# arcosoph/nanowakeword

Hardware: AMD Instinct MI355X
Metric: clips/sec (1 s @16 kHz PCM->logits) (higher is better)
Workload: dtype f32; 1 GPU; cnn head on (101,64) log-mel, batch=4096/GPU, 1 s 16 kHz mono int16 clips, 64-mel 25 ms/10 ms center frontend, fused STFT+mel HIP kernel, fp32; clips_per_gpu=4096, n_samples=16000, parallelism=batch-split x1

## Files before the change

### nanowakeword_amd/csrc/gemm_x3.hip

```cpp
#include <hip/hip_runtime.h>
#include <stdint.h>
#include <stdlib.h>
#include "layers.h"
#include "split_h2.h"

typedef float f32x16 __attribute__((ext_vector_type(16)));
typedef __bf16 bf16x8 __attribute__((ext_vector_type(8)));
typedef _Float16 f16x8 __attribute__((ext_vector_type(8)));
typedef _Float16 f16x2 __attribute__((ext_vector_type(2)));
typedef float f32x2 __attribute__((ext_vector_type(2)));
typedef float f32x4v __attribute__((ext_vector_type(4)));
typedef uint32_t u32x4v __attribute__((ext_vector_type(4)));

#ifdef X3_TRACE
__device__ unsigned long long x3_trace_buf[4 * 16 * 4];
#define X3_STAMP(kt_rel, ph)                                                                                        \
    if (blockIdx.x == 0 && blockIdx.y == 0 && blockIdx.z == 0 && (kt_rel) < 16 && (threadIdx.x & 63) == 0)        \
        x3_trace_buf[((threadIdx.x >> 6) * 16 + (kt_rel)) * 4 + (ph)] = __builtin_readcyclecounter();
#else
#define X3_STAMP(kt_rel, ph)
#endif
namespace {
constexpr int X3_BM = 128;
template <bool H2> struct X3A { static constexpr int NT = H2 ? 2 : 3, ROW = 64 * NT + 16; };

__device__ __forceinline__ float x3_sigmoid(float v) {
    return __builtin_amdgcn_rcpf(1.0f + __builtin_amdgcn_exp2f(-1.4426950408889634f * v));
}
template <int ACT>
__device__ __forceinline__ float x3_act(float v) {
    if (ACT == ACT_RELU) return fmaxf(v, 0.0f);
    if (ACT == ACT_GELU) return nww_gelu(v);
    if (ACT == ACT_SILU) return v * x3_sigmoid(v);
    if (ACT == ACT_SIGMOID) return x3_sigmoid(v);
    return v;
}

__device__ __forceinline__ void split3(float x, uint32_t& hi, uint32_t& mid, uint32_t& lo) {
    hi = __float_as_uint(x) & 0xffff0000u;
    const float r = x - __uint_as_float(hi);
    mid = __float_as_uint(r) & 0xffff0000u;
    lo = __float_as_uint(r - __uint_as_float(mid));
}
__device__ __forceinline__ uint32_t pack_hi16(uint32_t a, uint32_t b) { return __builtin_amdgcn_perm(b, a, 0x07060302u); }
template <bool H2>
__device__ __forceinline__ void x3_products(const uint4* a, const uint4* w, f32x16& acc) {
    if (H2) {
        const f16x8 ah = __builtin_bit_cast(f16x8, a[0]), al = __builtin_bit_cast(f16x8, a[1]);
        const f16x8 wh = __builtin_bit_cast(f16x8, w[0]), wl = __builtin_bit_cast(f16x8, w[1]);
        acc = __builtin_amdgcn_mfma_f32_32x32x16_f16(al, wh, acc, 0, 0, 0);
        acc = __builtin_amdgcn_mfma_f32_32x32x16_f16(ah, wl, acc, 0, 0, 0);
        acc = __builtin_amdgcn_mfma_f32_32x32x16_f16(ah, wh, acc, 0, 0, 0);
    } else {
        const bf16x8 ah = __builtin_bit_cast(bf16x8, a[0]), am = __builtin_bit_cast(bf16x8, a[1]), al = __builtin_bit_cast(bf16x8, a[H2 ? 1 : 2]);
        const bf16x8 wh = __builtin_bit_cast(bf16x8, w[0]), wm = __builtin_bit_cast(bf16x8, w[1]), wl = __builtin_bit_cast(bf16x8, w[H2 ? 1 : 2]);
        acc = __builtin_amdgcn_mfma_f32_32x32x16_bf16(am, wm, acc, 0, 0, 0);
        acc = __builtin_amdgcn_mfma_f32_32x32x16_bf16(ah, wl, acc, 0, 0, 0);
        acc = __builtin_amdgcn_mfma_f32_32x32x16_bf16(al, wh, acc, 0, 0, 0);
        acc = __builtin_amdgcn_mfma_f32_32x32x16_bf16(ah, wm, acc, 0, 0, 0);
        acc = __builtin_amdgcn_mfma_f32_32x32x16_bf16(am, wh, acc, 0, 0, 0);
        acc = __builtin_amdgcn_mfma_f32_32x32x16_bf16(ah, wh, acc, 0, 0, 0);
    }
}
}

__global__ void __launch_bounds__(256) split_weights_x3_kernel(const float* __restrict__ W, uint16_t* __restrict__ out,
                                                               int N, int K, int KB) {
    const size_t idx = (size_t)blockIdx.x * 256 + threadIdx.x;
    const size_t total = (size_t)N * KB * 16;
    if (idx >= total) return;
    const int kk = (int)(idx & 15);
    const size_t nb = idx >> 4;
    const int kb = (int)(nb % KB), n = (int)(nb / KB);
    const int k = kb * 16 + kk;
    const float x = k < K ? W[(size_t)n * K + k] : 0.0f;
    uint32_t hi, mid, lo;
    split3(x, hi, mid, lo);
    uint16_t* o = out + nb * 48 + kk;
    o[0] = (uint16_t)(hi >> 16); o[16] = (uint16_t)(mid >> 16); o[32] = (uint16_t)(lo >> 16);
}

__global__ void __launch_bounds__(256) split_weights_h2_kernel(const float* __restrict__ W, uint16_t* __restrict__ out,
                                                               int N, int K, int KB, float scale) {
    const size_t idx = (size_t)blockIdx.x * 256 + threadIdx.x;
    const size_t total = (size_t)N * KB * 16;
    if (idx >= total) return;
    const int kk = (int)(idx & 15);
    const size_t nb = idx >> 4;
    const int kb = (int)(nb % KB), n = (int)(nb / KB);
    const int k = kb * 16 + kk;
    const float x = k < K ? W[(size_t)n * K + k] * scale : 0.0f;
    uint32_t hi, lo;
    nww_split2h(x, 0.0f, hi, lo);
    uint16_t* o = out + nb * 32 + kk;
    o[0] = (uint16_t)hi; o[16] = (uint16_t)lo;
}

template <int CB, int NST, int ACT, bool H2>
__global__ void __launch_bounds__(256) __attribute__((amdgpu_num_vgpr(184))) gemm_x3_kernel(GemmArgs g) {
    constexpr int NT = X3A<H2>::NT, X3_ROW = X3A<H2>::ROW, PB = 2 * NT;
    { float agpr_hint = 0.0f; asm volatile("; mfma accumulators in AGPRs" : "+a"(agpr_hint)); }
    constexpr int BN = 32 * CB;
    constexpr int WPIECES = BN * 2 * PB;
    constexpr int WLD = (WPIECES + 255) / 256;
    extern __shared__ __attribute__((aligned(16))) unsigned char smem[];
    auto As = [&](int) { return smem; };
    auto Ws = [&](int) { return smem + X3_BM * X3_ROW; };
    const int tid = threadIdx.x, lane = tid & 63, wave = tid >> 6;
    const int i = lane & 31, h = lane >> 5;
    const int bxi = blockIdx.x, byi = blockIdx.y, bzi = blockIdx.z;
    const int bm = bxi * X3_BM, bn = byi * BN;
    const int KT = (g.K + 31) >> 5, KB = 2 * KT;
    int kt_begin = 0, kt_end = KT;
    if (g.splitk > 1) {
        const int kc = (KT + g.splitk - 1) / g.splitk;
        kt_begin = bzi * kc;
        kt_end = min(KT, kt_begin + kc);
    }
    const uint4* Wx = reinterpret_cast<const uint4*>(g.Wx3);

    const int lr = tid >> 3, lq = tid & 7;
    const float* arow[4];
#pragma unroll
    for (int q = 0; q < 4; ++q)
        arow[q] = g.a_blocked ? g.A + ((size_t)(bm >> 7) * g.a_blocked * 128 + lr + 32 * q) * 32 + 4 * lq
                              : g.A + (size_t)min(bm + lr + 32 * q, g.M - 1) * g.lda + 4 * lq;
    const int a_kstep = g.a_blocked ? 128 * 32 : 32;
    constexpr int AQ = (NST > 1 && CB == 1) ? 2 : 4;
    struct Stage { f32x4v a[AQ]; u32x4v w[WLD]; };
    auto gload = [&](int kt, Stage& st) {
        const int k = kt * 32 + 4 * lq;
        const size_t a_off = k + 4 <= g.K ? (size_t)kt * a_kstep : 0;
#pragma unroll
        for (int q = 0; q < AQ; ++q) {
            st.a[q] = *reinterpret_cast<const f32x4v*>(arow[q] + a_off);
        }
#pragma unroll
        for (int j = 0; j < WLD; ++j) {
            const int p = tid + 256 * j;
            if (WPIECES % 256 == 0 || p < WPIECES) {
                const int row = p / (2 * PB), c = p - row * (2 * PB);
                const int n = min(bn + row, g.N - 1);
                const int kb = 2 * kt + c / PB;
                st.w[j] = *reinterpret_cast<const u32x4v*>(Wx + ((size_t)n * KB + kb) * PB + (c % PB));
            }
        }
    };
    const float a_scale = H2 ? g.a_scale : 1.0f;
    const float a_lim = H2 ? (g.a_clamp > 0.0f ? g.a_clamp * a_scale : 65504.0f) : 0.0f;
    auto lstore = [&](int buf, const Stage& st) {
#pragma unroll
        for (int q = 0; q < AQ; ++q) {
            unsigned char* d = As(buf) + (lr + 32 * q) * X3_ROW + 8 * lq;
            if (H2) {
                uint32_t h0, l0, h1, l1;
                nww_split2h(__builtin_amdgcn_fmed3f(st.a[q][0] * a_scale, -a_lim, a_lim), __builtin_amdgcn_fmed3f(st.a[q][1] * a_scale, -a_lim, a_lim), h0, l0);
                nww_split2h(__builtin_amdgcn_fmed3f(st.a[q][2] * a_scale, -a_lim, a_lim), __builtin_amdgcn_fmed3f(st.a[q][3] * a_scale, -a_lim, a_lim), h1, l1);
                *reinterpret_cast<uint2*>(d) = make_uint2(h0, h1);
                *reinterpret_cast<uint2*>(d + 64) = make_uint2(l0, l1);
            } else {
                uint32_t hi[4], mid[4], lo[4];
                split3(st.a[q][0], hi[0], mid[0], lo[0]); split3(st.a[q][1], hi[1], mid[1], lo[1]);
                split3(st.a[q][2], hi[2], mid[2], lo[2]); split3(st.a[q][3], hi[3], mid[3], lo[3]);
                *reinterpret_cast<uint2*>(d) = make_uint2(pack_hi16(hi[0], hi[1]), pack_hi16(hi[2], hi[3]));
                *reinterpret_cast<uint2*>(d + 64) = make_uint2(pack_hi16(mid[0], mid[1]), pack_hi16(mid[2], mid[3]));
                *reinterpret_cast<uint2*>(d + 128) = make_uint2(pack_hi16(lo[0], lo[1]), pack_hi16(lo[2], lo[3]));
            }
        }
#pragma unroll
        for (int j = 0; j < WLD; ++j) {
            const int p = tid + 256 * j;
            if (WPIECES % 256 == 0 || p < WPIECES) {
                const int row = p / (2 * PB), c = p - row * (2 * PB);
                const int cp = c % PB;
                *reinterpret_cast<u32x4v*>(Ws(buf) + row * X3_ROW + (cp >> 1) * 64 + (c / PB) * 32 + (cp & 1) * 16) = st.w[j];
            }
        }
    };

    f32x16 acc[CB];
#pragma unroll
    for (int c = 0; c < CB; ++c)
#pragma unroll
        for (int r = 0; r < 16; ++r) acc[c][r] = 0.0f;

    Stage st[NST];
#pragma unroll
    for (int q = 0; q < NST; ++q) gload(min(kt_begin + q, kt_end - 1), st[q]);
    const bool has_rows = bm + wave * 32 < g.M;
    const int a_off = (wave * 32 + i) * X3_ROW + 16 * h, w_off = i * X3_ROW + 16 * h;
    auto multiply = [&]() {
#pragma unroll
        for (int kk = 0; kk < 2; ++kk) {
            const unsigned char* ap = As(0) + a_off + 32 * kk;
            uint4 af[NT];
#pragma unroll
            for (int t = 0; t < NT; ++t) af[t] = *reinterpret_cast<const uint4*>(ap + 64 * t);
#pragma unroll
            for (int c = 0; c < CB; ++c) {
                const unsigned char* wp = Ws(0) + w_off + c * 32 * X3_ROW + 32 * kk;
                uint4 wf[NT];
#pragma unroll
                for (int t = 0; t < NT; ++t) wf[t] = *reinterpret_cast<const uint4*>(wp + 64 * t);
                x3_products<H2>(af, wf, acc[c]);
            }
        }
    };
    for (int kt = kt_begin; kt < kt_end; kt += NST) {
#pragma unroll
        for (int q = 0; q < NST; ++q) {
            if (kt + q < kt_end) {
                X3_STAMP(kt + q - kt_begin, 0)
                __syncthreads();
                X3_STAMP(kt + q - kt_begin, 1)
                lstore(0, st[q]);
                __syncthreads();
                X3_STAMP(kt + q - kt_begin, 2)
            }
            gload(min(kt + q + NST, kt_end - 1), st[q]);
            if (kt + q < kt_end && (NST == 1 || has_rows)) multiply();
            X3_STAMP(kt + q - kt_begin, 3)
        }
    }

    const int m0 = bm + wave * 32;
    if (m0 >= g.M) return;
    if (H2) {
        const float c_scale = g.c_scale;
#pragma unroll
        for (int c = 0; c < CB; ++c)
#pragma unroll
            for (int r = 0; r < 16; ++r) acc[c][r] *= c_scale;
    }
#pragma unroll
    for (int c = 0; c < CB; ++c) {
        const int n = bn + c * 32 + i;
        if (n >= g.N) continue;
        if (g.splitk > 1) {
            float* part = g.splitk_ws + (size_t)bzi * g.M * g.N;
#pragma unroll
            for (int r = 0; r < 16; ++r) {
                const int m = m0 + (r & 3) + 8 * (r >> 2) + 4 * h;
                if (m < g.M) part[(size_t)m * g.N + n] = acc[c][r];
            }
            continue;
        }
        const float bias = g.bias ? g.bias[n] : 0.0f;
        const float al2 = g.alpha ? g.alpha[n] : 1.0f, be2 = g.alpha ? g.beta[n] : 0.0f;
        float* cp = g.C + (size_t)(m0 + 4 * h) * g.ldc + n;
        const float* rp = g.res ? g.res + (size_t)(m0 + 4 * h) * g.ldres + n : nullptr;
        const bool full = m0 + 32 <= g.M;
        auto finish = [&](float a) {
            float v = a + bias;
            v = v * al2 + be2;
            return x3_act<ACT>(v);
        };
        if (full && !rp) {
#pragma unroll
            for (int r = 0; r < 16; ++r) cp[(size_t)((r & 3) + 8 * (r >> 2)) * g.ldc] = finish(acc[c][r]);
        } else if (full) {
#pragma unroll
            for (int r = 0; r < 16; ++r) {
                const size_t ro = (size_t)((r & 3) + 8 * (r >> 2));
                cp[ro * g.ldc] = rp[ro * g.ldres] + g.rscale * finish(acc[c][r]);
            }
        } else {
#pragma unroll
            for (int r = 0; r < 16; ++r) {
                const int mo = (r & 3) + 8 * (r >> 2);
                if (m0 + 4 * h + mo < g.M) {
                    float v = finish(acc[c][r]);
                    if (rp) v = rp[(size_t)mo * g.ldres] + g.rscale * v;
                    cp[(size_t)mo * g.ldc] = v;
                }
            }
        }
    }
}

constexpr int CH_NW = 8, CH_TPW = 4;
template <bool H2>
__global__ void __launch_bounds__(64 * CH_NW) gemm_x3_chain_kernel(GemmArgs g) {
    constexpr int NT = X3A<H2>::NT, PB = 2 * NT;
    const float a_scale = H2 ? g.a_scale : 1.0f, c_scale = H2 ? g.c_scale : 1.0f;
    const float a_lim = H2 ? (g.a_clamp > 0.0f ? g.a_clamp * a_scale : 65504.0f) : 0.0f;
    __shared__ __attribute__((aligned(16))) float4 hand[4 * 64];
    const int lane = threadIdx.x & 63, wave = __builtin_amdgcn_readfirstlane((int)(threadIdx.x >> 6));
    const int i = lane & 31, h = lane >> 5;
    const int bm = blockIdx.x * 32, bn = blockIdx.y * 32;
    const int KT = (g.K + 31) >> 5, KB = 2 * KT;
    const int kc = (KT + g.splitk - 1) / g.splitk;
    const int kt_begin = blockIdx.z * kc, kt_end = min(KT, kt_begin + kc);
    const int mrow = min(bm + i, g.M - 1);
    const uint4* wrow = reinterpret_cast<const uint4*>(g.Wx3) + (size_t)min(bn + i, g.N - 1) * KB * PB + h;
    const float* abase = g.a_blocked ? g.A + ((size_t)(mrow >> 7) * g.a_blocked * 128 + (mrow & 127)) * 32 + 8 * h
                                     : g.A + (size_t)mrow * g.lda + 8 * h;
    const size_t a_kstep = g.a_blocked ? 128 * 32 : 32;

    f32x16 acc;
#pragma unroll
    for (int r = 0; r < 16; ++r) acc[r] = 0.0f;
    if (kt_begin >= kt_end) {
        if (wave == 0 && bn + i < g.N) {
            float* part = g.splitk_ws + (size_t)blockIdx.z * g.M * g.N;
#pragma unroll
            for (int r = 0; r < 16; ++r) {
// ... 84 lines not shown

hipError_t launch_split_weights_h2(const float* W, void* out, int N, int K, float scale, hipStream_t s) {
    const int KB = 2 * ((K + 31) / 32);
    const size_t total = (size_t)N * KB * 16;
    hipLaunchKernelGGL(split_weights_h2_kernel, dim3((unsigned)((total + 255) / 256)), dim3(256), 0, s, W,
                       reinterpret_cast<uint16_t*>(out), N, K, KB, scale);
    return hipGetLastError();
}

hipError_t launch_split_weights_x3(const float* W, void* out, int N, int K, hipStream_t s) {
    const int KB = 2 * ((K + 31) / 32);
    const size_t total = (size_t)N * KB * 16;
    hipLaunchKernelGGL(split_weights_x3_kernel, dim3((unsigned)((total + 255) / 256)), dim3(256), 0, s, W,
                       reinterpret_cast<uint16_t*>(out), N, K, KB);
    return hipGetLastError();
}

static int x3_pick_cb(int N) {
    int best = 2;
    long best_cost = -1;
    for (int cb = 2; cb <= 6; ++cb) {
        const long tiles = (N + 32 * cb - 1) / (32 * cb);
        const long cost = tiles * 32 * cb * 8 - cb;
        if (best_cost < 0 || cost < best_cost) { best_cost = cost; best = cb; }
    }
    return best;
}

bool gemm_x3_usable(const GemmArgs& g) {
    return g.Wx3 != nullptr && g.N >= 32 && g.K >= 32 && (g.K % 4 == 0) && (g.lda % 4 == 0) && (!g.a_blocked || g.K % 32 == 0) &&
           ((reinterpret_cast<uintptr_t>(g.A) & 15) == 0);
}

hipError_t launch_gemm_x3(const GemmArgs& g, hipStream_t s) {
    const int sk = (g.splitk > 1 && g.splitk_ws) ? g.splitk : 1;
    GemmArgs a = g;
    a.splitk = sk;
    const bool h2 = a.h2 != 0;
    const size_t row_b = h2 ? X3A<true>::ROW : X3A<false>::ROW;
#define X3_GO1(CBV, NSTV, ACTV, H2V, GRID, LDSB)                                                                   \
    {                                                                                                              \
        hipError_t e = nww_allow_lds(reinterpret_cast<const void*>(gemm_x3_kernel<CBV, NSTV, ACTV, H2V>), LDSB);   \
        if (e != hipSuccess) return e;                                                                             \
        hipLaunchKernelGGL((gemm_x3_kernel<CBV, NSTV, ACTV, H2V>), GRID, dim3(256), LDSB, s, a);                   \
    }
#define X3_GO(CBV, NSTV, ACTV, GRID, LDSB)                                                                         \
    if (h2) X3_GO1(CBV, NSTV, ACTV, true, GRID, LDSB) else X3_GO1(CBV, NSTV, ACTV, false, GRID, LDSB)
#define X3_ACT(CBV, NSTV, GRID, LDSB)                                                                              \
    switch (sk > 1 ? (int)ACT_NONE : a.act) {       \
        case ACT_RELU: X3_GO(CBV, NSTV, ACT_RELU, GRID, LDSB) break;                                               \
        case ACT_GELU: X3_GO(CBV, NSTV, ACT_GELU, GRID, LDSB) break;                                               \
        case ACT_SILU: X3_GO(CBV, NSTV, ACT_SILU, GRID, LDSB) break;                                               \
        case ACT_SIGMOID: X3_GO(CBV, NSTV, ACT_SIGMOID, GRID, LDSB) break;                                         \
        default: X3_GO(CBV, NSTV, ACT_NONE, GRID, LDSB) break;                                                     \
    }
    if (g.M <= 64 && sk > 1 && g.K % 8 == 0) {
        if (h2) hipLaunchKernelGGL(gemm_x3_chain_kernel<true>, dim3((g.M + 31) / 32, (g.N + 31) / 32, sk), dim3(64 * CH_NW), 0, s, a);
        else hipLaunchKernelGGL(gemm_x3_chain_kernel<false>, dim3((g.M + 31) / 32, (g.N + 31) / 32, sk), dim3(64 * CH_NW), 0, s, a);
        return hipGetLastError();
    }
    if (g.M <= 64) {
        dim3 grid1(1, (g.N + 31) / 32, sk);
        const size_t lds1 = (size_t)(X3_BM + 32) * row_b;
        X3_ACT(1, 8, grid1, lds1)
        return hipGetLastError();
    }
    int cb = x3_pick_cb(g.N);
    {
        const long mt = (g.M + X3_BM - 1) / X3_BM, pad = (long)((g.N + 32 * cb - 1) / (32 * cb)) * 32 * cb;
        if (mt * ((g.N + 32 * cb - 1) / (32 * cb)) * sk < 256) {
            int pick = cb;
            for (int c = cb - 1; c >= 2; --c) {
                const long tiles = (g.N + 32 * c - 1) / (32 * c);
                if (tiles * 32 * c != pad) continue;
                pick = c;
                if (mt * tiles * sk >= 256) break;
            }
            cb = pick;
        }
    }
    const int bn = 32 * cb;
    dim3 grid((g.M + X3_BM - 1) / X3_BM, (g.N + bn - 1) / bn, sk);
    const size_t lds = (size_t)(X3_BM + bn) * row_b;
    switch (cb) {
        case 2: X3_ACT(2, 1, grid, lds) break;
        case 3: X3_ACT(3, 1, grid, lds) break;
        case 4: X3_ACT(4, 1, grid, lds) break;
        case 5: X3_ACT(5, 1, grid, lds) break;
        case 6: X3_ACT(6, 1, grid, lds) break;
        default: return hipErrorInvalidValue;
    }
#undef X3_ACT
#undef X3_GO
#undef X3_GO1
    return hipGetLastError();
}
```

### nanowakeword_amd/csrc/layers.h

```cpp
#pragma once
#include <hip/hip_runtime.h>
#include "rnn.h"

#include <map>
#include <mutex>
#include <utility>
inline hipError_t nww_allow_lds(const void* func, size_t bytes) {
    if (bytes <= 64 * 1024) return hipSuccess;
    static std::mutex mu;
    static std::map<std::pair<int, const void*>, size_t> done;
    int dev = 0;
    hipError_t e = hipGetDevice(&dev);
    if (e != hipSuccess) return e;
    std::lock_guard<std::mutex> lk(mu);
    size_t& cur = done[std::make_pair(dev, func)];
    if (bytes > cur) {
        e = hipFuncSetAttribute(func, hipFuncAttributeMaxDynamicSharedMemorySize, (int)bytes);
        if (e != hipSuccess) return e;
        cur = bytes;
    }
    return hipSuccess;
}

__device__ __forceinline__ float nww_silu(float v) {
    return v * __builtin_amdgcn_rcpf(1.0f + __builtin_amdgcn_exp2f(v * -1.4426950408889634f));
}

__device__ __forceinline__ float nww_gelu(float x) {
    const float t = fabsf(x);
    float r = -1.7879411728927153e-08f;
    r = fmaf(r, t, 5.763639592260006e-07f);
    r = fmaf(r, t, -7.931240361358505e-06f);
    r = fmaf(r, t, 5.882469122298062e-05f);
    r = fmaf(r, t, -0.00021966989152133465f);
    r = fmaf(r, t, -0.00012137762678321451f);
    r = fmaf(r, t, 0.0070888083428144455f);
    r = fmaf(r, t, -0.05253036320209503f);
    r = fmaf(r, t, -0.45919492840766907f);
    r = fmaf(r, t, -1.151106595993042f);
    const float h = __builtin_amdgcn_exp2f(fmaxf(fmaf(r, t, -1.0f), -126.0f));
    return x * (x >= 0.0f ? 1.0f - h : h);
}

enum NwwAct { ACT_RELU = 0, ACT_GELU = 1, ACT_SILU = 2, ACT_NONE = 3, ACT_SIGMOID = 4, ACT_SWISH = 2 };

struct GemmArgs {
    const float* A; int lda;
    const float* W;
    float* C; int ldc;
    int M, N, K;
    const float* bias; const float* alpha; const float* beta;
    int act;
    const float* res; int ldres; float rscale;
    int splitk = 0; float* splitk_ws = nullptr;
    bool defer_reduce = false;
    const void* Wx3 = nullptr;
    int h2 = 0; float a_scale = 1.0f, c_scale = 1.0f, a_clamp = 0.0f;
    int a_blocked = 0;
    const float* A2 = nullptr; int lda2 = 0; const float* W2 = nullptr; int K2 = 0;
    const float* alpha2 = nullptr; const float* beta2 = nullptr;
};
size_t gemm_x3_weight_bytes(int N, int K);
hipError_t launch_split_weights_x3(const float* W, void* out, int N, int K, hipStream_t s);
hipError_t launch_split_weights_h2(const float* W, void* out, int N, int K, float scale, hipStream_t s);
bool gemm_x3_usable(const GemmArgs& g);
bool gemm_writes_partials(const GemmArgs& g);
hipError_t launch_gemm_x3(const GemmArgs& g, hipStream_t s);
int gemm_recommended_splitk(long long M, int N, int K, int cu_count);
hipError_t launch_gemm(const GemmArgs& g, hipStream_t s);

struct Conv3Args {
    const float* in; const float* w; const float* bias; const float* alpha; const float* beta;
    float* out; int B, Cin, Cout, H, W; int act; int pool;
    int nhwc_out = 0;
};
hipError_t launch_conv3x3(const Conv3Args& a, hipStream_t s);

hipError_t launch_dwconv3x3_nhwc(const float* in, const float* wt, float* d_out, float* xs_out, int B, int C, int H,
                                 int W, int sh, int sw, hipStream_t s, int act16 = 0, float out_mul = 1.0f);
hipError_t launch_layernorm_parts(const float* parts, int nparts, size_t part_stride, const float* in_bias, float* y, const float* w,
                                  const float* b, int R, int D, int act, hipStream_t s);
hipError_t launch_layernorm(const float* x, float* y, const float* w, const float* b, int R, int D, int act,
                            hipStream_t s);
hipError_t launch_mean_mid(const float* in, float* out, int B, int L, int D, hipStream_t s, int act16 = 0, float unscale = 1.0f);
hipError_t launch_ln_mean(const float* x, float* out, const float* w, const float* b, int B, int L, int D, hipStream_t s);
hipError_t launch_avgpool(const float* in, float* out, int BC, int H, int W, int kh, int kw, int sh, int sw, int oh,
                          int ow, hipStream_t s);
hipError_t launch_unary(const float* x, float* y, size_t n, int act, hipStream_t s);
hipError_t launch_scale_add_pe(float* x, const float* pe, int B, int T, int D, float scale, hipStream_t s);
hipError_t launch_glu(const float* in, float* out, int R, int D, hipStream_t s);
hipError_t launch_branch_merge(float* x, const float* a, const float* c, const float* z, size_t n, hipStream_t s);
hipError_t launch_dwconv1d_bn_swish(const float* x, const float* w , const float* bias, const float* alpha,
                                    const float* beta, float* y, int B, int T, int D, int K, hipStream_t s);
hipError_t launch_mha_core(const float* qkv, float* out, int B, int T, int D, int n_head, hipStream_t s);
bool mha_mfma_supported(int T, int D, int n_head);
hipError_t launch_mha_mfma(const float* qkv, float* out, int B, int T, int D, int n_head, int cus, hipStream_t s, int head_major = 0);
bool mha_head_dim_supported(int head_dim);
bool mha_h2_supported(int T, int D, int n_head);
hipError_t launch_mha_h2(const float* qkv, float* out, int B, int T, int D, int n_head, int cus, hipStream_t s, int head_major = 0);
hipError_t launch_crnn_seq(const float* in, float* out, int B, int C, int H, int W, hipStream_t s);
hipError_t launch_transpose_planes(const float* in, float* out, int B, int R, int C, hipStream_t s);

struct TailArgs {
    const float* x; int Kin;
    const float *We, *be; int E;
    const float *W0, *b0, *w3, *b3;
    float *emb, *logits, *probs;
    int B, act;
    const float* parts = nullptr; int nparts = 0; size_t part_stride = 0;
    const float *in_bias = nullptr, *in_alpha = nullptr, *in_beta = nullptr; int in_act = 0;
    unsigned int* done_flag = nullptr; unsigned int done_seq = 0;
    const float *ln0_w = nullptr, *ln0_b = nullptr;
    int n_mid = 0;
    const float *mid_W[4] = {nullptr, nullptr, nullptr, nullptr}, *mid_b[4] = {nullptr, nullptr, nullptr, nullptr};
    const float *mid_lnw[4] = {nullptr, nullptr, nullptr, nullptr}, *mid_lnb[4] = {nullptr, nullptr, nullptr, nullptr};
    int cu_count = 256;
};
bool tail_supported(int Kin, int E);
bool tail_batch_runs(int B, int Kin, int E, bool dnn_body, int nparts);
hipError_t launch_classifier_tail(const TailArgs& a, hipStream_t s);
```

### nanowakeword_amd/csrc/nww_internal.h

```cpp
#pragma once
#include <hip/hip_runtime.h>
#include <algorithm>
#include <atomic>
#include <cmath>
#include <cstdarg>
#include <cstdio>
#include <cstdlib>
#include <cstring>
#include <functional>
#include <map>
#include <string>
#include <vector>

#include "../../include/nww.h"
#include "fe_tables.h"
#include "stream_plan.h"
#include "stream_pool.h"
#include "raw_plan.h"
#include "plan_host.h"
#include "frontend.h"
#include "layers.h"
#include "trunk.h"
#include "ffn_x3.h"
#include "lin_x3.h"
// ... 127 lines not shown
    std::vector<std::vector<hipEvent_t>> prof_runs;
    std::vector<std::vector<int>> prof_ids;
    std::vector<hipEvent_t> event_pool;
    std::vector<double> prof_ms;
    std::vector<int> prof_cnt;
};


int nww_fail(nww_handle* h, int code, const char* fmt, ...);
std::string& nww_create_err();
void nww_prof_mark(nww_handle* h, hipStream_t s, int id_of_next);
void nww_prof_begin(nww_handle* h);
int nww_check_run(nww_handle* h, int B);
int nww_ensure_ws(nww_handle* h, int B, int N);
struct RunOpts {
    bool x_frames_major = false;
    unsigned int* done_flag = nullptr;
    unsigned int done_seq = 0;
    bool* done_armed = nullptr;
    const HopView* hop = nullptr;
};
int nww_run_head(nww_handle* h, const float* d_x, int B, float* d_logits, float* d_probs, hipStream_t s, const RunOpts& o = RunOpts());
int nww_frontend_on_dev(nww_handle* h, const int16_t* d_pcm, int B, int N, float* d_db, float* d_mel, int frames_major, hipStream_t s,
                        int* frames_out, size_t row_stride = 0, const Fe2Sub* sub = nullptr);
int nww_forward_pcm_on_dev(nww_handle* h, const int16_t* d_pcm, int B, int N, float* d_logits, float* d_probs, hipStream_t s,
                           size_t row_stride = 0, const RunOpts& o = RunOpts());
int nww_h2d_small(nww_handle* h, void* dst, const void* src, size_t bytes, hipStream_t s);
int nww_copy_out(nww_handle* h, int B, float* logits, float* probs, float* emb, hipStream_t s);
void nww_recording_free(nww_handle* h);
long long nww_rec_count(long long n_samples, int W, int hop);
int nww_rec_grow(nww_handle* h, void** p, size_t* cap, size_t bytes);
int nww_rec_forward_on_dev(nww_handle* h, const int16_t* d_pcm, long long n_samples, int W, int hop, int max_batch, float* d_logits, float* d_probs,
                           hipStream_t s);
int nww_pool_push_check(nww_handle* h, const int32_t* idx, int32_t n, const void* chunk, bool* done);
int nww_pool_push_on_dev(nww_handle* h, const int32_t* idx, int n, const int16_t* d_chunk, float* d_logits, float* d_probs, hipStream_t s,
                         const PoolEntry** tab_out = nullptr, int* m_out = nullptr);
void nww_cascade_free(nww_handle* h);
void nww_build_spec(nww_handle* h);
void balance_channel_gains(nww_handle* h);
void fold_batchnorms(nww_handle* h);
void transpose_depthwise(nww_handle* h);
void transpose_e2e_filters(nww_handle* h);
void fold_quartznet(nww_handle* h);
void fold_raw_frontend(nww_handle* h);
void fold_raw_backbone(nww_handle* h);
int upload_weight_arena(nww_handle* h);
int build_frontend_tables(nww_handle* h);
inline bool nww_raw_head(const nww_config& c) { return c.head_type == NWW_HEAD_E2E_QUARTZNET || c.head_type == NWW_HEAD_E2E_CNN; }
inline int nww_row_floats(const nww_config& c) { return nww_raw_head(c) ? c.in_cols : c.n_mels; }
inline int nww_pcm_rows(const nww_handle* h, int N) {
    if (!nww_raw_head(h->cfg)) return fe_num_frames(h->fe, N);
    int L = N;
    for (int i = 0; i < h->cfg.n_blocks; ++i) L = raw_conv_rows(L, i == 0 ? 16 : 4);
    return L < 1 ? -1 : L;
}
struct ClipRows { int T, rows, cols; bool fits; };
inline ClipRows nww_clip_rows(const nww_handle* h, int N) {
    const nww_config& c = h->cfg;
    const int T = nww_pcm_rows(h, N);
    const int rows = c.mel_major_features ? c.n_mels : T, cols = nww_raw_head(c) ? c.in_cols : c.mel_major_features ? T : c.n_mels;
    return {T, rows, cols, T > 0 && rows == c.in_rows && cols == c.in_cols};
}
inline int nww_fail_short_clip(nww_handle* h, int N) {
    if (nww_raw_head(h->cfg)) return nww_fail(h, NWW_ERR_INVALID, "a clip needs at least one sample (got %d)", N);
    return nww_fail(h, NWW_ERR_INVALID, "clip of %d samples is too short for n_fft=%d (center=%d)", N, h->fe.n_fft, h->fe.center);
}
int nww_window_plan(nww_handle* h, int W, int hop, int level, HopPlan& p);
struct RawCnnLayer { int cin, cout, sA, sB; };
inline const RawCnnLayer* nww_raw_cnn_layers() {
    static const RawCnnLayer L[4] = {{1, 24, 2, 1}, {24, 48, 2, 2}, {48, 64, 2, 2}, {64, 96, 1, 1}};
    return L;
}
inline std::string nww_quartznet_prefix(const nww_config& c) { return nww_raw_head(c) ? "model.backbone." : "model."; }
struct QnBlock { int cin, cout, k; };
inline std::vector<QnBlock> nww_quartznet_blocks(const nww_config& c) {
    std::vector<QnBlock> v;
    int cin = c.in_cols;
    for (int i = 0; i < c.n_crnn_channels && i < 4; ++i)
        for (int r = 0; r < (c.quartznet_kr[i] >> 16); ++r) { v.push_back({cin, c.crnn_channels[i], c.quartznet_kr[i] & 0xFFFF}); cin = c.crnn_channels[i]; }
    return v;
}

struct Knobs {
    int trunk, conv_mfma, conv3_x3, gemm_x3, lin_x3, ffn_fused, attn_fused, merge_fused, qn_fused, raw_fused, conv2s_x3, rnn_ih_fused, mha_mfma, bc_front, bc_chain, tail;
    int stream_inc;
    int rec_shared;
    int f16_range_log2;
};
const Knobs& nww_knobs();

#define fail nww_fail
#define HIP_TRY(h, expr)                                                                             \
    do {                                                                                             \
        hipError_t e_ = (expr);                                                                      \
        if (e_ != hipSuccess) return fail(h, NWW_ERR_HIP, "%s failed: %s", #expr, hipGetErrorString(e_)); \
    } while (0)
```

### nanowakeword_amd/csrc/nww_plan.hip

```cpp
#include "nww_internal.h"
#include "bc_chain.h"

const Knobs& nww_knobs() {
    static const Knobs k = [] {
        auto env = [](const char* name, int d) { const char* e = getenv(name); return e ? atoi(e) : d; };
        Knobs r;
        r.trunk = env("NWW_TRUNK", 1); r.conv_mfma = env("NWW_CONV_MFMA", 1); r.conv3_x3 = env("NWW_CONV3_X3", 1);
        r.gemm_x3 = env("NWW_GEMM_X3", 1); r.lin_x3 = env("NWW_LIN_X3", 1); r.ffn_fused = env("NWW_FFN_FUSED", 1);
        r.attn_fused = env("NWW_ATTN_FUSED", 1); r.merge_fused = env("NWW_MERGE_FUSED", 1); r.qn_fused = env("NWW_QN_FUSED", 1); r.raw_fused = env("NWW_RAW_FUSED", 1); r.conv2s_x3 = env("NWW_CONV2S_X3", 1); r.rnn_ih_fused = env("NWW_RNN_IH_FUSED", 1); r.mha_mfma = env("NWW_MHA_MFMA", 1); r.bc_front = env("NWW_BC_FRONT", 1);
        r.bc_chain = env("NWW_BC_CHAIN", 1); r.tail = env("NWW_TAIL", 1); r.stream_inc = env("NWW_STREAM_INC", 3); r.rec_shared = env("NWW_REC_SHARED", 1);
        r.f16_range_log2 = env("NWW_F16_RANGE_LOG2", 16);
        return r;
    }();
    return k;
}
double f16_range_factor() { return std::ldexp(1.0, nww_knobs().f16_range_log2); }

namespace {

enum : int { BUF_X = -1, BUF_EMB = -2, BUF_HID = -3, BUF_LOGITS = -4, BUF_NONE = 99 };

struct PlanCtx {
    nww_handle* h;
    const float* W(const std::string& k) const {
        auto it = h->tensors.find(k);
        return it == h->tensors.end() || !it->second.loaded ? nullptr : h->d_weights + it->second.dev_off;
    }
    void need(int buf, size_t floats_per_clip) {
        if (h->buf_per_clip[buf] < floats_per_clip) h->buf_per_clip[buf] = floats_per_clip;
    }
    void add(const std::string& name, std::function<hipError_t(Run&)> fn) { h->plan.push_back({name, std::move(fn)}); }
    void pop_last() { if (!h->plan.empty()) h->plan.pop_back(); }
    std::string tail_name; int tail_in = BUF_NONE, tail_K = 0; const float *tail_W = nullptr, *tail_b = nullptr;
    struct DnnBody { bool on = false; const float *ln0_w = nullptr, *ln0_b = nullptr; int n_mid = 0; const float* mid[4][4] = {}; } dnn;
    struct Packs {
        nww_handle* h;
        std::vector<void*> held;
        explicit Packs(PlanCtx& p) : h(p.h) {}
        Packs(const Packs&) = delete;
        ~Packs() { for (void* d : held) (void)hipFree(d); }
        void* alloc(size_t bytes) { void* d = nullptr; if (hipMalloc(&d, bytes) != hipSuccess) return nullptr; held.push_back(d); return d; }
        template <class Launch> void* pack(size_t bytes, Launch&& launch) {
            void* d = alloc(bytes);
            if (d && launch(d) != hipSuccess) { held.pop_back(); (void)hipFree(d); d = nullptr; }
            return d;
        }
        void commit() { h->packed_weights.insert(h->packed_weights.end(), held.begin(), held.end()); held.clear(); }
    };
    template <class Launch> void* pack_one(size_t bytes, Launch&& launch) { Packs pk(*this); void* d = pk.pack(bytes, launch); pk.commit(); return d; }
};

std::vector<float> f16_fetch(nww_handle* h, const float* d, size_t n) {
    if (!d) return std::vector<float>(n, 0.0f);
    const uintptr_t a = reinterpret_cast<uintptr_t>(d), a0 = reinterpret_cast<uintptr_t>(h->d_weights);
    const size_t size = h->h_weights.size(), off = a >= a0 ? (size_t)(a - a0) / sizeof(float) : size + 1;
    if ((a - a0) % sizeof(float) != 0 || off > size || n > size - off) {
        if (h->plan_error.empty()) h->plan_error = "plan-time read of " + std::to_string(n) + " weights outside the weight arena";
        return std::vector<float>(n, 0.0f);
    }
    return std::vector<float>(h->h_weights.begin() + off, h->h_weights.begin() + off + n);
}
double f16_ln_bound(nww_handle* h, const float* w, const float* b, int D) {
    const auto hw = f16_fetch(h, w, D), hb = f16_fetch(h, b, D);
    double bound = 0.0;
    for (int k = 0; k < D; ++k) bound = std::fmax(bound, std::sqrt((double)D) * std::fabs((double)hw[k]) + std::fabs((double)hb[k]));
    return bound;
}
bool f16_all_nonneg(nww_handle* h, const float* d, int n) {
    for (float v : f16_fetch(h, d, n)) if (!(v >= 0.0f)) return false;
    return true;
}

const F16Range F16_FEATURES{NWW_F16_FEATURE_BOUND, 32.0};

inline const float* src(Run& r, int id) { return id == BUF_X ? r.x : id == BUF_EMB ? r.emb : id == BUF_HID ? r.hid : r.buf[id]; }
inline float* dst(Run& r, int id) { return id == BUF_EMB ? r.emb : id == BUF_HID ? r.hid : id == BUF_LOGITS ? r.logits : r.buf[id]; }

struct GemmOpts {
    const float *alpha = nullptr, *beta = nullptr;
    int res_id = BUF_NONE; float rscale = 1.f;
    bool* a_blocked_inout = nullptr;
    bool feeds_tail = false, feeds_ln = false;
    F16Range a_range; bool a_bound_assumed = false;
};
void add_gemm(PlanCtx& p, const std::string& name, int in_id, int out_id, int rows_per_clip, int N, int K,
              const float* W, const float* bias, int act, const GemmOpts& o = GemmOpts{}) {
    const double a_bound = o.a_range.ok() ? o.a_range.bound : 0.0;
    const int tail_E = p.h->cfg.embedding_dim;
    if (out_id >= 0) p.need(out_id, (size_t)rows_per_clip * N);
    const int x3_mode = nww_knobs().gemm_x3;
    const bool small_square = N <= 160 && K > 64 && K <= 160;
    const bool use_x3 = p.h->conv_products != 0 &&
                        (x3_mode == 2 ? (N >= 32 && K >= 32)
                         : x3_mode == 3 ? (K >= 4096 && N >= 64 && N <= 256)
                         : (x3_mode == 1 && N >= 64 && K >= 32 && !small_square));
    const void* wx3 = nullptr;
    float h2_as = 0.0f, h2_ws = 0.0f;
    if (use_x3 && p.h->f16 && a_bound > 0.0) {
        const auto hW = f16_fetch(p.h, W, (size_t)N * K);
        bool rows_ok = true;
        const int nch = (int)o.a_range.ch.size();
        if (nch > 0 && K % nch == 0) {
            const int per = K / nch;
            const F16Rows m = f16_rows_moments(N, K, [&](int q, int co) { return hW[(size_t)co * K + q]; }, [&](int q) { return q / per; }, o.a_range.ch);
            rows_ok = f16_rows_ok(a_bound, m) && f16_rows_weights_ok(m, K);
        }
        h2_as = rows_ok ? f16_scale(a_bound) : 0.0f;
        if (h2_as > 0.0f) h2_ws = f16_wscale(hW);
    }
    const bool h2_req = h2_as > 0.0f && h2_ws > 0.0f;
    if (use_x3) {
        const X3Key key{W, h2_req ? 1 : 0, h2_req ? h2_ws : 0.0f};
        auto it = p.h->x3_weights.find(key);
        if (it == p.h->x3_weights.end()) {
            void* d = nullptr;
            if (hipMalloc(&d, gemm_x3_weight_bytes(N, K)) == hipSuccess &&
                (h2_req ? launch_split_weights_h2(W, d, N, K, h2_ws, p.h->own_stream) : launch_split_weights_x3(W, d, N, K, p.h->own_stream)) == hipSuccess)
                it = p.h->x3_weights.emplace(key, d).first;
            else if (d) (void)hipFree(d);
        }
        if (it != p.h->x3_weights.end()) wx3 = it->second;
    }
    const bool h2 = h2_req && wx3 != nullptr;
    if (h2 && o.a_bound_assumed && in_id == BUF_X) p.h->clamps_features = true;
    const int a_blocked = (o.a_blocked_inout && *o.a_blocked_inout && wx3 && K % 32 == 0 && rows_per_clip == 1) ? K / 32 : 0;
    if (o.a_blocked_inout) *o.a_blocked_inout = a_blocked != 0;
    if (K >= 2048 && (size_t)16 * rows_per_clip * N > p.h->splitk_per_clip) p.h->splitk_per_clip = (size_t)16 * rows_per_clip * N;
    p.add("gemm:" + name + (h2 && wx3 ? " [f16x3]" : ""), [=](Run& r) {
        GemmArgs g;
        g.A = src(r, in_id); g.lda = K; g.W = W; g.C = dst(r, out_id); g.ldc = N;
        g.M = r.B * rows_per_clip; g.N = N; g.K = K; g.bias = bias; g.alpha = o.alpha; g.beta = o.beta; g.act = act;
        g.res = o.res_id == BUF_NONE ? nullptr : src(r, o.res_id); g.ldres = N; g.rscale = o.rscale;
        g.Wx3 = wx3;
        if (h2) { g.h2 = 1; g.a_scale = h2_as; g.c_scale = 1.0f / (h2_as * h2_ws); g.a_clamp = o.a_bound_assumed ? (float)a_bound : 0.0f; }
        g.a_blocked = a_blocked;
        g.splitk = gemm_recommended_splitk(g.M, N, K, r.cu_count);
        if (wx3 && x3_mode != 2 && K >= 2048) { g.splitk = K >= 8192 ? K / 800 : K / 512; if (g.splitk > 16) g.splitk = 16; if (g.splitk < 1) g.splitk = 1; }
        g.splitk_ws = r.splitk_ws;
        if (g.splitk > 1 && (size_t)g.splitk * g.M * N > r.splitk_floats) g.splitk = 1;
        r.deferred.active = false;
        const bool partials = g.splitk > 1 && g.splitk_ws && gemm_writes_partials(g);
        if (o.feeds_tail && partials && !g.res && (g.M <= 8 || tail_batch_runs(g.M, N, tail_E, false, g.splitk))) {
            g.defer_reduce = true;
            r.deferred.active = true; r.deferred.out_id = out_id; r.deferred.parts = g.splitk; r.deferred.stride = (size_t)g.M * N;
            r.deferred.bias = bias; r.deferred.alpha = o.alpha; r.deferred.beta = o.beta; r.deferred.act = act;
        }
        if (o.feeds_ln && partials && !g.res && !o.alpha && act == ACT_NONE && N <= 256) {
            g.defer_reduce = true;
            r.deferred.active = true; r.deferred.out_id = out_id; r.deferred.parts = g.splitk; r.deferred.stride = (size_t)g.M * N;
            r.deferred.bias = bias; r.deferred.alpha = nullptr; r.deferred.beta = nullptr; r.deferred.act = ACT_NONE;
        }
        return launch_gemm(g, r.stream);
    });
}

enum LinEpi : int { LIN_BIAS = 0, LIN_RES = 1, LIN_GLU = 2, LIN_RES_TAB = 3 };
struct LinOpts {
    int epi = LIN_BIAS, res_id = BUF_NONE; float rscale = 1.f; const float* res_tab = nullptr;
    const float *ln_w = nullptr, *ln_b = nullptr;
    int qkv_T = 0, qkv_dh = 0;
};
bool add_lin_x3(PlanCtx& p, const std::string& name, int in_id, int out_id, int rows_per_clip, int N, int K, const float* W,
                const float* bias, const LinOpts& o = LinOpts{}) {
    if (!nww_knobs().lin_x3 || p.h->conv_products != 6 || !lin_x3_supported(K, N, true)) return false;
    if (o.ln_w && o.epi != LIN_GLU && !(o.epi == LIN_BIAS && lin_x3_ln_plain_supported(K))) return false;
    const int parts = o.epi == LIN_GLU ? 2 : 1;
    float ws = 0.0f;
    if (p.h->f16) ws = f16_wscale(f16_fetch(p.h, W, (size_t)parts * N * K));
    const bool h2 = ws > 0.0f;
    if (!lin_x3_supported(K, N, h2)) return false;
    const int terms = h2 ? 2 : 3;
    void* packed = p.pack_one(lin_x3_packed_bytes(K, N, parts, terms), [&](void* d) { return launch_lin_x3_pack(W, bias, d, K, N, parts, N, p.h->own_stream, terms, h2 ? ws : 1.0f); });
    if (!packed) return false;
    p.need(out_id, (size_t)rows_per_clip * N);
    const float w_un = h2 ? 1.0f / ws : 1.0f;
    p.add("lin_x3:" + name + (h2 ? " [f16x3]" : ""), [=](Run& r) {
        LinArgs a;
        a.x = src(r, in_id); a.ldx = K; a.out = dst(r, out_id); a.ldc = N;
        a.res = o.res_tab ? o.res_tab : o.res_id == BUF_NONE ? nullptr : src(r, o.res_id); a.ldres = N; a.rscale = o.rscale;
        a.ln_w = o.ln_w; a.ln_b = o.ln_b; a.packed = static_cast<const unsigned char*>(packed);
        a.M = r.B * rows_per_clip; a.N = N; a.qkv_T = o.qkv_T; a.qkv_dh = o.qkv_dh;
        a.h2 = h2 ? 1 : 0; a.w_un = w_un;
        return launch_lin_x3(a, K, o.epi, o.ln_w != nullptr, r.stream);
    });
    return true;
}

void add_linear(PlanCtx& p, const std::string& name, int in_id, int out_id, int rows_per_clip, int N, int K, const float* W,
                const float* bias, int res_id = BUF_NONE, float rscale = 1.f) {
    LinOpts lo; lo.epi = res_id == BUF_NONE ? LIN_BIAS : LIN_RES; lo.res_id = res_id; lo.rscale = rscale;
    GemmOpts go; go.res_id = res_id; go.rscale = rscale;
    if (!add_lin_x3(p, name, in_id, out_id, rows_per_clip, N, K, W, bias, lo))
        add_gemm(p, name, in_id, out_id, rows_per_clip, N, K, W, bias, ACT_NONE, go);
}

void set_tail(PlanCtx& p, const std::string& name, int in_id, int K, const float* W, const float* b) {
    p.tail_name = name; p.tail_in = in_id; p.tail_K = K; p.tail_W = W; p.tail_b = b;
}

void add_conv(PlanCtx& p, const std::string& name, int in_id, int out_id, int Cin, int Cout, int H, int W,
              const float* w, const float* bias, const float* alpha, const float* beta, int act, int pool, int nhwc_out = 0) {
    const int Ho = pool ? H / 2 : H, Wo = pool ? W / 2 : W;
    p.need(out_id, (size_t)Cout * Ho * Wo);
    p.add("conv3x3:" + name, [=](Run& r) {
        Conv3Args a{src(r, in_id), w, bias, alpha, beta, dst(r, out_id), r.B, Cin, Cout, H, W, act, pool};
        a.nhwc_out = nhwc_out;
        return launch_conv3x3(a, r.stream);
    });
}

static int trunk_fits(int C1, int H, int W) { int per_cu = 0; return trunk_pick_strips(C1, H, W, &per_cu); }
struct TrunkOpts { const bool* out_blocked = nullptr; F16Range in_range; F16Range* out_range = nullptr; };
bool add_trunk(PlanCtx& p, const std::string& name, int in_id, int out_id, int C1, int C2, int H, int W,
               const float* w1, const float* b1, const float* al1, const float* be1, const float* w2,
               const float* b2, const float* al2, const float* be2, int act, const TrunkOpts& o = TrunkOpts{}) {
    if (o.out_range) *o.out_range = F16Range{};
    const double in_bound = o.in_range.ok() ? o.in_range.bound : 0.0;
    if (!nww_knobs().trunk || C1 != 16 || C2 != 32 || H < 4 || W < 4 || trunk_fits(C1, H, W) == 0) return false;
// ... 1272 lines not shown
```

Before: 9.369 million clips/s.

## Ping-pong two 256-thread tiles per 512-thread block in split-K x3 GEMM

Result: faster. 9.508 million clips/s (median of 6 runs) (+1.5%).

```diff
diff --git a/nanowakeword_amd/csrc/gemm_x3.hip b/nanowakeword_amd/csrc/gemm_x3.hip
--- a/nanowakeword_amd/csrc/gemm_x3.hip
+++ b/nanowakeword_amd/csrc/gemm_x3.hip
@@ -13,7 +13,7 @@
 typedef uint32_t u32x4v __attribute__((ext_vector_type(4)));
 
 #ifdef X3_TRACE
-__device__ unsigned long long x3_trace_buf[4 * 16 * 4];
+__device__ unsigned long long x3_trace_buf[8 * 16 * 4];
 #define X3_STAMP(kt_rel, ph)                                                                                        \
     if (blockIdx.x == 0 && blockIdx.y == 0 && blockIdx.z == 0 && (kt_rel) < 16 && (threadIdx.x & 63) == 0)        \
         x3_trace_buf[((threadIdx.x >> 6) * 16 + (kt_rel)) * 4 + (ph)] = __builtin_readcyclecounter();
@@ -96,19 +96,22 @@
     o[0] = (uint16_t)hi; o[16] = (uint16_t)lo;
 }
 
-template <int CB, int NST, int ACT, bool H2>
-__global__ void __launch_bounds__(256) __attribute__((amdgpu_num_vgpr(184))) gemm_x3_kernel(GemmArgs g) {
+template <int CB, int NST, int ACT, bool H2, bool PP = false>
+__global__ void __launch_bounds__(PP ? 512 : 256) __attribute__((amdgpu_num_vgpr(184))) gemm_x3_kernel(GemmArgs g) {
     constexpr int NT = X3A<H2>::NT, X3_ROW = X3A<H2>::ROW, PB = 2 * NT;
     { float agpr_hint = 0.0f; asm volatile("; mfma accumulators in AGPRs" : "+a"(agpr_hint)); }
     constexpr int BN = 32 * CB;
     constexpr int WPIECES = BN * 2 * PB;
     constexpr int WLD = (WPIECES + 255) / 256;
     extern __shared__ __attribute__((aligned(16))) unsigned char smem[];
-    auto As = [&](int) { return smem; };
-    auto Ws = [&](int) { return smem + X3_BM * X3_ROW; };
-    const int tid = threadIdx.x, lane = tid & 63, wave = tid >> 6;
+    const int hf = PP ? __builtin_amdgcn_readfirstlane((int)(threadIdx.x >> 8)) : 0;
+    unsigned char* const region = smem + hf * ((X3_BM + BN) * X3_ROW);
+    auto As = [&](int) { return region; };
+    auto Ws = [&](int) { return region + X3_BM * X3_ROW; };
+    const int tid = threadIdx.x & 255, lane = tid & 63;
+    const int wave = PP ? __builtin_amdgcn_readfirstlane(tid >> 6) : tid >> 6;
     const int i = lane & 31, h = lane >> 5;
-    const int bxi = blockIdx.x, byi = blockIdx.y, bzi = blockIdx.z;
+    const int bxi = PP ? 2 * blockIdx.x + hf : blockIdx.x, byi = blockIdx.y, bzi = blockIdx.z;
     const int bm = bxi * X3_BM, bn = byi * BN;
     const int KT = (g.K + 31) >> 5, KB = 2 * KT;
     int kt_begin = 0, kt_end = KT;
@@ -123,7 +126,7 @@
     const float* arow[4];
 #pragma unroll
     for (int q = 0; q < 4; ++q)
-        arow[q] = g.a_blocked ? g.A + ((size_t)(bm >> 7) * g.a_blocked * 128 + lr + 32 * q) * 32 + 4 * lq
+        arow[q] = g.a_blocked ? g.A + ((size_t)min(bm >> 7, (g.M - 1) >> 7) * g.a_blocked * 128 + lr + 32 * q) * 32 + 4 * lq
                               : g.A + (size_t)min(bm + lr + 32 * q, g.M - 1) * g.lda + 4 * lq;
     const int a_kstep = g.a_blocked ? 128 * 32 : 32;
     constexpr int AQ = (NST > 1 && CB == 1) ? 2 : 4;
@@ -206,6 +209,7 @@
             }
         }
     };
+    if (PP && hf) __syncthreads();
     for (int kt = kt_begin; kt < kt_end; kt += NST) {
 #pragma unroll
         for (int q = 0; q < NST; ++q) {
@@ -214,14 +218,16 @@
                 __syncthreads();
                 X3_STAMP(kt + q - kt_begin, 1)
                 lstore(0, st[q]);
+                if (PP) gload(min(kt + q + NST, kt_end - 1), st[q]);
                 __syncthreads();
                 X3_STAMP(kt + q - kt_begin, 2)
             }
-            gload(min(kt + q + NST, kt_end - 1), st[q]);
-            if (kt + q < kt_end && (NST == 1 || has_rows)) multiply();
+            if (!PP) gload(min(kt + q + NST, kt_end - 1), st[q]);
+            if (kt + q < kt_end && ((NST == 1 && !PP) || has_rows)) multiply();
             X3_STAMP(kt + q - kt_begin, 3)
         }
     }
+    if (PP && !hf) __syncthreads();
 
     const int m0 = bm + wave * 32;
     if (m0 >= g.M) return;
@@ -472,6 +478,12 @@
     const int bn = 32 * cb;
     dim3 grid((g.M + X3_BM - 1) / X3_BM, (g.N + bn - 1) / bn, sk);
     const size_t lds = (size_t)(X3_BM + bn) * row_b;
+    if (a.pp && h2 && a.a_blocked && cb == 4 && sk > 1) {
+        hipError_t e = nww_allow_lds(reinterpret_cast<const void*>(gemm_x3_kernel<4, 1, ACT_NONE, true, true>), 2 * lds);
+        if (e != hipSuccess) return e;
+        hipLaunchKernelGGL((gemm_x3_kernel<4, 1, ACT_NONE, true, true>), dim3((grid.x + 1) / 2, grid.y, sk), dim3(512), 2 * lds, s, a);
+        return hipGetLastError();
+    }
     switch (cb) {
         case 2: X3_ACT(2, 1, grid, lds) break;
         case 3: X3_ACT(3, 1, grid, lds) break;
diff --git a/nanowakeword_amd/csrc/layers.h b/nanowakeword_amd/csrc/layers.h
--- a/nanowakeword_amd/csrc/layers.h
+++ b/nanowakeword_amd/csrc/layers.h
@@ -57,6 +57,7 @@
     const void* Wx3 = nullptr;
     int h2 = 0; float a_scale = 1.0f, c_scale = 1.0f, a_clamp = 0.0f;
     int a_blocked = 0;
+    int pp = 0;
     const float* A2 = nullptr; int lda2 = 0; const float* W2 = nullptr; int K2 = 0;
     const float* alpha2 = nullptr; const float* beta2 = nullptr;
 };
diff --git a/nanowakeword_amd/csrc/nww_internal.h b/nanowakeword_amd/csrc/nww_internal.h
--- a/nanowakeword_amd/csrc/nww_internal.h
+++ b/nanowakeword_amd/csrc/nww_internal.h
@@ -233,7 +233,7 @@
 }
 
 struct Knobs {
-    int trunk, conv_mfma, conv3_x3, gemm_x3, lin_x3, ffn_fused, attn_fused, merge_fused, qn_fused, raw_fused, conv2s_x3, rnn_ih_fused, mha_mfma, bc_front, bc_chain, tail;
+    int trunk, conv_mfma, conv3_x3, gemm_x3, lin_x3, ffn_fused, attn_fused, merge_fused, qn_fused, raw_fused, conv2s_x3, rnn_ih_fused, mha_mfma, bc_front, bc_chain, tail, gemm_pp;
     int stream_inc;
     int rec_shared;
     int f16_range_log2;
diff --git a/nanowakeword_amd/csrc/nww_plan.hip b/nanowakeword_amd/csrc/nww_plan.hip
--- a/nanowakeword_amd/csrc/nww_plan.hip
+++ b/nanowakeword_amd/csrc/nww_plan.hip
@@ -8,7 +8,7 @@
         r.trunk = env("NWW_TRUNK", 1); r.conv_mfma = env("NWW_CONV_MFMA", 1); r.conv3_x3 = env("NWW_CONV3_X3", 1);
         r.gemm_x3 = env("NWW_GEMM_X3", 1); r.lin_x3 = env("NWW_LIN_X3", 1); r.ffn_fused = env("NWW_FFN_FUSED", 1);
         r.attn_fused = env("NWW_ATTN_FUSED", 1); r.merge_fused = env("NWW_MERGE_FUSED", 1); r.qn_fused = env("NWW_QN_FUSED", 1); r.raw_fused = env("NWW_RAW_FUSED", 1); r.conv2s_x3 = env("NWW_CONV2S_X3", 1); r.rnn_ih_fused = env("NWW_RNN_IH_FUSED", 1); r.mha_mfma = env("NWW_MHA_MFMA", 1); r.bc_front = env("NWW_BC_FRONT", 1);
-        r.bc_chain = env("NWW_BC_CHAIN", 1); r.tail = env("NWW_TAIL", 1); r.stream_inc = env("NWW_STREAM_INC", 3); r.rec_shared = env("NWW_REC_SHARED", 1);
+        r.bc_chain = env("NWW_BC_CHAIN", 1); r.tail = env("NWW_TAIL", 1); r.stream_inc = env("NWW_STREAM_INC", 3); r.rec_shared = env("NWW_REC_SHARED", 1); r.gemm_pp = env("NWW_GEMM_PP", 1);
         r.f16_range_log2 = env("NWW_F16_RANGE_LOG2", 16);
         return r;
     }();
@@ -134,6 +134,7 @@
         g.Wx3 = wx3;
         if (h2) { g.h2 = 1; g.a_scale = h2_as; g.c_scale = 1.0f / (h2_as * h2_ws); g.a_clamp = o.a_bound_assumed ? (float)a_bound : 0.0f; }
         g.a_blocked = a_blocked;
+        g.pp = nww_knobs().gemm_pp;
         g.splitk = gemm_recommended_splitk(g.M, N, K, r.cu_count);
         if (wx3 && x3_mode != 2 && K >= 2048) { g.splitk = K >= 8192 ? K / 800 : K / 512; if (g.splitk > 16) g.splitk = 16; if (g.splitk < 1) g.splitk = 1; }
         g.splitk_ws = r.splitk_ws;
```
